# balisujohn/tortoise.cpp

Measured on AMD Instinct MI355X. Metric: audio-seconds/sec end-to-end (AR+diffusion+vocoder), 16 cands x 80 steps, higher is better.
Workload: dtype f16 MFMA inputs / f32 accumulate (diffusion, vocoder convs); f32 weights, f16 KV (AR)

## Files before the change

### tortoise.cpp_amd/csrc/api.cpp

```cpp
#include "common.h"
#include <sched.h>
#include <cctype>
#include <cmath>
#include <algorithm>
#include <chrono>
#include <fstream>
#include <new>

namespace tts {
int ar_begin(tts_ctx *, const int32_t *, int, const float *, int, int);
int ar_begin_groups(tts_ctx *, const int32_t *, const int *, int, const float *, int n_voices, const int *voice_of, const int *, int);
int ar_latents_group(tts_ctx *, int, const int32_t *, int, float *);
int ar_prefill(tts_ctx *, float *);
int ar_step(tts_ctx *, const int32_t *, int, float *, int mode);
const int32_t *ar_host_lists(tts_ctx *);
const float *ar_fetch_logits_row(tts_ctx *, int);
int ar_batch(const tts_ctx *);
int ar_latents(tts_ctx *, const int32_t *, int, int, float *);
int ar_layers(const tts_ctx *);
float *ar_host_logits(tts_ctx *);
int diff_layers(const tts_ctx *);
int diff_forward(tts_ctx *, const float *, int, const float *, int, int, float *);
int diff_sample(tts_ctx *, const float *, const int32_t *, int, int, const float *, int, float *);
int diff_sample_voices(tts_ctx *, const float *, const int32_t *, int, const float *, int, const int32_t *, int, const float *, int, float *);
// ... 113 lines not shown
  for (hipEvent_t e : c->ev_pool) (void)hipEventDestroy(e);
  if (c->ev0) (void)hipEventDestroy(c->ev0);
  if (c->ev1) (void)hipEventDestroy(c->ev1);
  if (c->stream) (void)hipStreamDestroy(c->stream);
  if (c->load_stream) (void)hipStreamDestroy(c->load_stream);
  delete c;
}

int tts_version(void) { return TTS_API_VERSION; }

const char *tts_last_error(const tts_ctx *c) { return c ? c->err.c_str() : "no context (no HIP device?)"; }

int tts_set_option(tts_ctx *c, const char *key, double value) {
  if (!c || !key) return TTS_ERR_ARG;
  std::string k(key);
  if (k == "gn_eps") c->gn_eps = (float)value;
  else if (k == "ggml_lut") c->ggml_lut = value != 0;
  else if (k.rfind("prof_only:", 0) == 0) {
    if (value != 0) c->prof_filter.push_back(k.substr(10));
    else c->prof_filter.clear();
  }
  else if (k == "device_topk") c->device_topk = value != 0;
  else if (k == "sampler_threads") {
    if (c->sampler_pool) { sampler_pool_free(c->sampler_pool); c->sampler_pool = nullptr; }
    c->sampler_threads = value < 0 ? -1 : (int)value;
  }
  else if (k == "share_uncond") c->share_uncond = value != 0;
  else if (k == "prof_stride") c->prof_stride = value < 1 ? 1 : (int)value;
  else if (k == "diff_graph") c->diff_graph = value != 0;
  else if (k == "dec_f32_mfma") c->dec_f32_mfma = value != 0;
  else if (k == "attn_f32") c->attn_f32 = value != 0;
  else if (k == "attn_proj_f16") c->attn_proj_f16 = value != 0;
  else if (k == "proj_dual_b") c->proj_dual_b = value != 0;
  else if (k == "gemm_wreg") c->gemm_wreg = value == 1 ? tts_ctx::GEMM_WREG_ALL : value == 2 ? 1 : value == 3 ? 2 : 0;
  else if (k == "lc_attn_f32") c->lc_attn_f32 = value != 0;
  else if (k == "latency_mode") c->latency_mode = value != 0;
  else if (k == "fp16_check") c->fp16_check = value != 0;
  else if (k == "rng_fast_normal") c->rng_fast_normal = value != 0;
  else if (k == "noise_pipeline") c->noise_pipeline = value != 0;
  else if (k == "load_device_pack") c->load_device_pack = value != 0;
  else if (k == "load_threads") c->load_threads = value < 0 ? 0 : value > 64 ? 64 : (int)value;
  else if (k == "attn_q64") c->attn_q64 = value < 0 ? 0 : value > 2 ? 2 : (int)value;
  else if (k == "hoist_integrator") c->hoist_integrator = value < 0 ? 0 : (int)value;
  else if (k == "attn_f32_drop") c->attn_f32_drop = (int)value & 7;
  else if (k == "ar_weights") {
    if (value != 0 && value != 1 && value != 2) return fail(c, TTS_ERR_ARG, "ar_weights: 0 (f32), 1 (fp16) or 2 (fp8 e4m3)");
    c->ar_weights = (int)value;
  }
  else if (k == "diff_sampler") {
    if (value != 0 && value != 1) return fail(c, TTS_ERR_ARG, "diff_sampler: 0 (ancestral DDPM) or 1 (DDIM)");
    c->diff_sampler = (int)value;
  }
  else if (k == "ddim_eta") {
    if (!(value >= 0 && value <= 1)) return fail(c, TTS_ERR_ARG, "ddim_eta: a value in [0, 1]");
    c->ddim_eta = value;
  }
  else if (k == "cond_free_k") {
    if (!std::isfinite(value) || value < 0 || !std::isfinite((float)value)) return fail(c, TTS_ERR_ARG, "cond_free_k: a finite value >= 0");
    c->cond_free_k = (float)value;
  }
  else if (k == "prof_eager_every") c->prof_eager_every = value < 1 ? 1 : (int)value;
  else if (k == "stream_cus") {
    if (c->device < 0) return fail(c, TTS_ERR_HIP, "host-only context: no stream");
    if (c->ar || c->diff || c->voc || c->clvp || c->venc || c->dcond) return fail(c, TTS_ERR_STATE, "stream_cus must be set before the models are loaded");
    (void)hipSetDevice(c->device);
    hipDeviceProp_t prop;
    if (hipGetDeviceProperties(&prop, c->device) != hipSuccess) return fail(c, TTS_ERR_HIP, "hipGetDeviceProperties failed");
// ... 435 lines not shown
```

### tortoise.cpp_amd/csrc/common.h

```cpp
#pragma once
#include "../../include/tortoise_mi355x.h"
#include <hip/hip_runtime.h>
#include <cstdarg>
#include <cstdint>
#include <cstdio>
#include <cstring>
#include <functional>
#include <map>
#include <memory>
#include <random>
#include <algorithm>
#include <atomic>
#include <condition_variable>
#include <mutex>
#include <new>
#include <string>
#include <thread>
#include <vector>

namespace tts {

struct HostTensor {
  std::vector<float> data;
  int64_t ne[4] = {1, 1, 1, 1};
// ... 67 lines not shown
  int device = 0;
  hipStream_t stream = nullptr;
  hipStream_t load_stream = nullptr;
  int stream_cus = 0;
  std::string err;
  float gn_eps = 1e-6f;
  int ggml_lut = 0;
  std::mt19937 generator;
  std::uniform_real_distribution<float> distribution{0.0, 1.0};
  std::normal_distribution<double> normal_distribution{0.0, 1.0};
  uint32_t seed_value = 0;
  tts::ArState *ar = nullptr;
  tts::DiffState *diff = nullptr;
  tts::VocState *voc = nullptr;
  tts::ClvpState *clvp = nullptr;
  tts::VoiceEncState *venc = nullptr;
  tts::DiffCondEncState *dcond = nullptr;
  tts::Tokenizer *tok = nullptr;
  tts::SamplerPool *sampler_pool = nullptr;
  int device_topk = 1;
  int time_mlp_retries = 0;
  int topk_fallbacks = 0;
  int sampler_threads = -1;
  bool share_uncond = true;
  int rng_shard_offset = 0, rng_shard_total = 0;
  std::vector<int32_t> stop_schedule;
  std::vector<int32_t> ar_stopped;
  bool prof_on = false;
  std::vector<std::string> prof_filter;
  int prof_stride = 1;
  int ar_weights = 0;
  int dec_f32_mfma = 0;
  int attn_f32 = 0;
  static constexpr int GEMM_WREG_ALL = 3;
  int gemm_wreg = GEMM_WREG_ALL;
  int proj_dual_b = 1;
  int attn_f32_drop = 0;
  int lc_attn_f32 = 1;
  int attn_proj_f16 = 0;
  int fp16_check = 0;
  int64_t fp16_bad_weights[2] = {0, 0};
  void *fp16_counts = nullptr;
  int rng_fast_normal = 1;
  int noise_pipeline = 1;
  int load_device_pack = 1;
  int load_threads = 0;
  int attn_q64 = 0;
  int hoist_integrator = 1;
  int latency_mode = 0;
  int diff_sampler = 0;
  double ddim_eta = 0;
  float cond_free_k = 2.0f;
  bool capturing = false;
  int diff_graph = 1;
  int prof_eager_every = 8;
  std::map<std::string, tts::ProfEntry> prof;
  std::vector<hipEvent_t> ev_pool;
  hipEvent_t ev0 = nullptr, ev1 = nullptr;
};

namespace tts {

int fail(tts_ctx *ctx, int code, const char *fmt, ...);

void rng_normal_fill(tts_ctx *ctx, float *dst, int64_t n);

struct PinnedPool {
// ... 178 lines not shown
```

### tortoise.cpp_amd/csrc/diffusion.hip

```cpp
#include "common.h"
#include "gemm_f16.h"
#include <algorithm>
#include <chrono>
#include <cmath>

namespace tts {

static constexpr int C = 1024, NHEAD = 16, XTC = 128 ;
static constexpr int LAT_MAX_ROWS = 2048;
static constexpr int HOIST_MAX_ROWS = 16384;

__device__ __forceinline__ float silu_dev(float x, int lut) {
  if (lut == 1) {
    float xr = __half2float(__float2half_rn(x));
    return __half2float(__float2half_rn(xr / (1.0f + expf(-xr))));
  }
  if (lut == 2) return x / (1.0f + expf(-x));
  return x * __builtin_amdgcn_rcpf(1.0f + __builtin_amdgcn_exp2f(x * -1.44269504088896f));
}

__global__ __launch_bounds__(256) void gn_stats_kernel(const float *__restrict__ x, const int *__restrict__ seq_start,
                                                       const int *__restrict__ seq_len, float eps, float2 *__restrict__ stats) {
  __shared__ float sh[8];
  const int grp = blockIdx.x, s = blockIdx.y, T = seq_len[s];
// ... 667 lines not shown
    const float xs = sc.sqrt_recip * xv;
    float x0 = xs - sc.sqrt_recipm1 * eps_g;
    x0 = fminf(fmaxf(x0, -1.0f), 1.0f);
    const float eps_h = (xs - x0) / sc.sqrt_recipm1;
    outv = d.c_x0 * x0 + d.c_eps * eps_h;
    if (!sc.is_last && d.sigma != 0.0f) {
      const float nz = noise ? noise[xi] : philox_normal(seed, stream0 + (uint32_t)s, e.philox_step, (uint32_t)(ch * T + t));
      outv = outv + d.sigma * nz;
    }
  }
  x[xi] = outv;
}

__global__ void philox_fill_kernel(float *__restrict__ x, int64_t n, uint64_t seed, uint32_t stream, uint32_t step) {
  int64_t i = (int64_t)blockIdx.x * blockDim.x + threadIdx.x;
  if (i < n) x[i] = philox_normal(seed, stream, step, (uint32_t)i);
}

__global__ void rows_to_ct_kernel(const float *__restrict__ net, int row0, int T, int nch, int ld, float *__restrict__ out) {
  int i = blockIdx.x * blockDim.x + threadIdx.x;
  if (i < nch * T) {
    int ch = i / T, t = i - ch * T;
    out[i] = net[(size_t)(row0 + t) * ld + ch];
  }
}

struct AttnDev {
  float *norm_g, *norm_b, *qkv_b, *proj_b, *bias_tab;
  __half *qkv_w, *proj_w;
  __half *qkv_wf;
  __half *proj_w_split;
  float proj_alpha;
};
struct ResDev { float *in_g, *in_b, *in_bias, *emb_w, *emb_b, *out_g, *out_b, *out_bias; __half *in_w, *out_w, *in_wf; };

struct Layout {
  int ns = 0, rows = 0;
  std::vector<int> start, len;
  DevBuf d_row_seq, d_row_t, d_start, d_len, d_chunk_seq;
  int build(tts_ctx *ctx, const std::vector<int> &lens) {
    has_seq_step = false; ss_step_stride = 0;
    ns = (int)lens.size();
    len = lens;
    start.resize(ns);
    int r = 8;
    for (int s = 0; s < ns; s++) { start[s] = r; r = (r + lens[s] + 1 + 7) & ~7; }
    rows = (r + 127) & ~127;
    std::vector<int> rs(rows, -1), rt(rows, 0);
    for (int s = 0; s < ns; s++)
      for (int t = 0; t < lens[s]; t++) { rs[start[s] + t] = s; rt[start[s] + t] = t; }
    TTS_HIP(ctx, d_row_seq.reserve(rows * 4)); TTS_HIP(ctx, d_row_t.reserve(rows * 4));
    TTS_HIP(ctx, d_start.reserve(ns * 4)); TTS_HIP(ctx, d_len.reserve(ns * 4));
    TTS_HIP(ctx, hipMemcpy(d_row_seq.p, rs.data(), rows * 4, hipMemcpyHostToDevice));
    TTS_HIP(ctx, hipMemcpy(d_row_t.p, rt.data(), rows * 4, hipMemcpyHostToDevice));
    TTS_HIP(ctx, hipMemcpy(d_start.p, start.data(), ns * 4, hipMemcpyHostToDevice));
    TTS_HIP(ctx, hipMemcpy(d_len.p, len.data(), ns * 4, hipMemcpyHostToDevice));
    std::vector<int> cs(rows / 8, -1);
    for (int s = 0; s < ns; s++)
      for (int t = 0; t < lens[s]; t++) cs[(start[s] + t) >> 3] = s;
    TTS_HIP(ctx, d_chunk_seq.reserve(rows / 8 * 4));
    TTS_HIP(ctx, hipMemcpy(d_chunk_seq.p, cs.data(), rows / 8 * 4, hipMemcpyHostToDevice));
    return TTS_OK;
  }
  int max_len() const { return len.empty() ? 0 : *std::max_element(len.begin(), len.end()); }
  DevBuf d_seq_step;
  int ss_step_stride = 0;
  bool has_seq_step = false;
// ... 100 lines not shown
    if (it->second.nelem() != nelem) {
      fail(ctx, TTS_ERR_FORMAT, "tensor '%s' has wrong size in model file: got %lld, expected %lld", name.c_str(),
           (long long)it->second.nelem(), (long long)nelem);
      return nullptr;
    }
    { std::lock_guard<std::mutex> lk(mu); used[name] = true; }
    return &it->second;
  }
  template <class T> int put(const std::vector<T> &h, T **dst) {
    void *p = nullptr;
    TTS_HIP(ctx, hipMalloc(&p, h.size() * sizeof(T)));
    { std::lock_guard<std::mutex> lk(mu); st->owned.push_back(p); }
    TTS_HIP(ctx, pin.upload(p, h.data(), h.size() * sizeof(T), ctx->load_stream));
    *dst = (T *)p;
    return TTS_OK;
  }
  int f32(const std::string &name, int64_t n, float **dst) {
    const HostTensor *t = get(name, n);
    if (!t) return TTS_ERR_FORMAT;
    return put(t->data, dst);
  }
  int conv16(const std::string &name, int cout, int cin, int k, int cout_pad, int cin_pad, __half **dst, __half **dst_frag = nullptr) {
    const HostTensor *t = get(name, (int64_t)cout * cin * k);
    if (!t) return TTS_ERR_FORMAT;
    std::vector<__half> h((size_t)cout_pad * k * cin_pad, __float2half(0.f));
    const float *w = t->data.data();
    for (int co = 0; co < cout; co++)
      for (int ci = 0; ci < cin; ci++)
        for (int tap = 0; tap < k; tap++)
          h[(size_t)co * k * cin_pad + (size_t)tap * cin_pad + ci] = __float2half_rn(w[((size_t)co * cin + ci) * k + tap]);
    if (dst_frag) {
      std::vector<__half> f(h.size());
      for (int n = 0; n < cout_pad; n++)
        for (int c = 0; c < cin_pad; c++) f[gemm_wfrag_index(n, c, cin_pad)] = h[(size_t)n * cin_pad + c];
      if (int r = put(f, dst_frag)) return r;
    }
    return put(h, dst);
  }
  int attn(const std::string &p, AttnDev &a) {
    int r;
    if ((r = f32(p + ".norm.weight", C, &a.norm_g))) return r;
    if ((r = f32(p + ".norm.bias", C, &a.norm_b))) return r;
    if ((r = conv16(p + ".qkv.weight", 3 * C, C, 1, 3 * C, C, &a.qkv_w, &a.qkv_wf))) return r;
    if ((r = f32(p + ".qkv.bias", 3 * C, &a.qkv_b))) return r;
    if ((r = conv16(p + ".proj_out.weight", C, C, 1, C, C, &a.proj_w))) return r;
    {
      const HostTensor *t = get(p + ".proj_out.weight", (int64_t)C * C);
      std::vector<__half> sp((size_t)C * 2 * C);
      float amax = 0.f;
      for (float v : t->data) amax = std::max(amax, std::fabs(v));
      if (!std::isfinite(amax)) { fail(ctx, TTS_ERR_FORMAT, "tensor '%s.proj_out.weight' holds a non-finite value", p.c_str()); return TTS_ERR_FORMAT; }
      int e = 14;
      while (e > -14 && std::ldexp(amax, e) >= 30000.0f) e--;
      const float scale = std::ldexp(1.0f, e);
      a.proj_alpha = 1.0f / scale;
      for (int n = 0; n < C; n++)
        for (int k = 0; k < C; k++) {
          const float w = t->data[(size_t)n * C + k] * scale;
          const __half hi = __float2half_rn(w);
          sp[(size_t)n * 2 * C + k] = hi;
          sp[(size_t)n * 2 * C + C + k] = __float2half_rn(w - __half2float(hi));
        }
      long long bad[2] = {0, 0};
      for (const __half &h : sp) {
        const float v = std::fabs(__half2float(h));
        if (!(v <= 65504.0f)) bad[0]++;
        else if (v > 60000.0f) bad[1]++;
      }
      if (bad[0] | bad[1]) { std::lock_guard<std::mutex> lk(mu); ctx->fp16_bad_weights[0] += bad[0]; ctx->fp16_bad_weights[1] += bad[1]; }
      if ((r = put(sp, &a.proj_w_split))) return r;
    }
    if ((r = f32(p + ".proj_out.bias", C, &a.proj_b))) return r;
    const HostTensor *t = get(p + ".relative_pos_embeddings.relative_attention_bias.weight", 32 * 16);
    if (!t) return TTS_ERR_FORMAT;
    std::vector<float> tab(16 * 128);
    for (int h = 0; h < 16; h++)
      for (int sgn = 0; sgn < 2; sgn++)
        for (int d = 0; d < 64; d++) {
          int bucket = sgn ? rel_bucket(0, d) : rel_bucket(d, 0);
          if (d == 0) bucket = rel_bucket(0, 0);
          tab[h * 128 + sgn * 64 + d] = t->data[(size_t)bucket * 16 + h] * 8.0f;
        }
    return put(tab, &a.bias_tab);
  }
  int res(const std::string &p, ResDev &w) {
    int r;
    if ((r = f32(p + ".in_layers.0.weight", C, &w.in_g))) return r;
    if ((r = f32(p + ".in_layers.0.bias", C, &w.in_b))) return r;
    if ((r = conv16(p + ".in_layers.2.weight", C, C, 1, C, C, &w.in_w, &w.in_wf))) return r;
    if ((r = f32(p + ".in_layers.2.bias", C, &w.in_bias))) return r;
    if ((r = f32(p + ".emb_layers.1.weight", 2 * C * C, &w.emb_w))) return r;
    if ((r = f32(p + ".emb_layers.1.bias", 2 * C, &w.emb_b))) return r;
    if ((r = f32(p + ".out_layers.0.weight", C, &w.out_g))) return r;
    if ((r = f32(p + ".out_layers.0.bias", C, &w.out_b))) return r;
    if ((r = conv16(p + ".out_layers.3.weight", C, C, 3, C, C, &w.out_w))) return r;
    if ((r = f32(p + ".out_layers.3.bias", C, &w.out_bias))) return r;
    return TTS_OK;
  }
};
}

int diff_load(tts_ctx *ctx, const char *path) {
  ctx->fp16_bad_weights[0] = ctx->fp16_bad_weights[1] = 0;
  WeightFile wf;
  std::string err;
  int rc = read_weight_file(path, wf, err);
  if (rc != TTS_OK) return fail(ctx, rc, "diffusion_model_load: %s", err.c_str());
  std::unique_ptr<DiffState> st(new DiffState());
  Loader ld{ctx, st.get(), wf, {}};
  while (wf.has("latent_conditioner." + std::to_string(st->n_lc + 1) + ".norm.weight")) st->n_lc++;
  while (wf.has("conditioning_timestep_integrator." + std::to_string(st->n_integ) + ".resblk.in_layers.0.weight")) st->n_integ++;
  while (wf.has("layers." + std::to_string(st->n_main) + ".resblk.in_layers.0.weight")) st->n_main++;
  while (wf.has("layers." + std::to_string(st->n_main + st->n_tail) + ".in_layers.0.weight")) st->n_tail++;
  st->lc_attn.resize(st->n_lc);
  st->integ_res.resize(st->n_integ); st->integ_attn.resize(st->n_integ);
  st->main_res.resize(st->n_main); st->main_attn.resize(st->n_main);
  st->tail_res.resize(st->n_tail);
  std::vector<std::function<int()>> jobs;
  DiffState *S = st.get();
#define J(x) jobs.emplace_back([&ld, S]() -> int { (void)S; return (x); })
  J(ld.f32("diffusion_conditioning_latent", 2 * C, &S->cond_latent));
  J(ld.f32("unconditioned_embedding", C, &S->uncond_emb));
  J(ld.conv16("latent_conditioner.0.weight", C, C, 3, C, C, &S->lc_w));
  J(ld.f32("latent_conditioner.0.bias", C, &S->lc_bias));
  for (int i = 0; i < st->n_lc; i++) jobs.emplace_back([&ld, S, i]() { return ld.attn("latent_conditioner." + std::to_string(i + 1), S->lc_attn[i]); });
  J(ld.f32("code_norm.weight", C, &S->code_g));
  J(ld.f32("code_norm.bias", C, &S->code_b));
  J(ld.f32("time_embed.0.weight", C * C, &S->te0_w)); J(ld.f32("time_embed.0.bias", C, &S->te0_b));
// ... 393 lines not shown
    return gemm(ctx, "diff_gemm", p, lay, 0, C);
  }
  if (!ctx->attn_proj_f16) {
    GemmArgs p = gemm_base(lay, wk.ATT16(), C, 2, C, w.proj_w_split, C, w.proj_b);
    p.custom_w = 1; p.ldw_ = 2 * C; p.w_off_[0] = 0; p.w_off_[1] = C;
    p.mode = st_out ? GEMM_OUT_F32_SCALED_STATS : GEMM_OUT_F32_SCALED; p.alpha = w.proj_alpha; p.outF = X; p.ldo = C; p.resid = X;
    p.st_out = st_out; p.st_stripe_ll = (int)st->gn_stripe_ll; p.chunk_seq = lay.d_chunk_seq.as<int>();
    p.dual_b = ctx->proj_dual_b;
    CHECK(gemm(ctx, "diff_gemm", p, lay, 0, C));
    DBG_SUM("attn proj", X, (size_t)lay.rows * C * 4);
    return TTS_OK;
  }
  GemmArgs p = gemm_base(lay, wk.ATT16(), C, 1, C, w.proj_w, C, w.proj_b);
  p.mode = st_out ? GEMM_OUT_F32_STATS : GEMM_OUT_F32; p.outF = X; p.ldo = C; p.resid = X;
  p.st_out = st_out; p.st_stripe_ll = (int)st->gn_stripe_ll; p.chunk_seq = lay.d_chunk_seq.as<int>();
  CHECK(gemm(ctx, "diff_gemm", p, lay));
  DBG_SUM("attn proj", X, (size_t)lay.rows * C * 4);
  return TTS_OK;
}

static int res_block(tts_ctx *ctx, DiffState *st, const Layout &lay, Work &wk, float *X, const ResDev &w, const float *ss,
                     const float *Xin = nullptr, const float *Hpre = nullptr, const long long *st_hpre = nullptr) {
  const float *xin = Xin ? Xin : X;
  const bool lat = st->lat && (Hpre ? st_hpre != nullptr : wk.st_x != nullptr);
  const long long *st_h = st_hpre;
  if (!Hpre) {
    long long *slot = lat ? st->new_stats_slot() : nullptr;
    CHECK(res_in_layers(ctx, st, lay, wk, xin, w, wk.H(), lat ? wk.st_x : nullptr, slot));
    Hpre = wk.H();
    st_h = slot;
  }
  DBG_SUM("res.out ss", ss, (size_t)2 * C * 4);
  DBG_SUM("res.out hpre", Hpre, (size_t)lay.rows * C * 4);
  CHECK(gn(ctx, st, lay, Hpre, lat ? st_h : nullptr, w.out_g, w.out_b, ss, 1, wk.A16(), w.out_w, (size_t)3 * C * C * 2));
  DBG_SUM("res.out gn", wk.A16(), (size_t)lay.rows * C * 2);
  GemmArgs c3 = gemm_base(lay, wk.A16(), C, 3, C, w.out_w, C, w.out_bias);
  long long *st_out = lat ? st->new_stats_slot() : nullptr;
  c3.mode = st_out ? GEMM_OUT_F32_STATS : GEMM_OUT_F32; c3.outF = X; c3.ldo = C; c3.resid = xin;
  c3.st_out = st_out; c3.st_stripe_ll = (int)st->gn_stripe_ll; c3.chunk_seq = lay.d_chunk_seq.as<int>();
  wk.st_x = st_out;
  CHECK(gemm(ctx, "diff_gemm", c3, lay));
  DBG_SUM("res.out conv", X, (size_t)lay.rows * C * 4);
  return TTS_OK;
}

template <int CTRL> __device__ __forceinline__ float lnk_dpp(float x) {
  return __int_as_float(__builtin_amdgcn_update_dpp(0, __float_as_int(x), CTRL, 0xf, 0xf, false));
}
__device__ __forceinline__ float wave_sum_dpp(float x) {
  auto a = __builtin_amdgcn_permlane32_swap(__float_as_uint(x), __float_as_uint(x), false, false);
  x = __uint_as_float(a[0]) + __uint_as_float(a[1]);
  auto b = __builtin_amdgcn_permlane16_swap(__float_as_uint(x), __float_as_uint(x), false, false);
  x = __uint_as_float(b[0]) + __uint_as_float(b[1]);
  x += lnk_dpp<0x128>(x);
  x += lnk_dpp<0x124>(x);
  x += lnk_dpp<0x122>(x);
  x += lnk_dpp<0x121>(x);
  return x;
}

static constexpr int LNK_COLS = 32;
static __global__ __launch_bounds__(1024) void linear_nk_kernel(const float *__restrict__ x, int ldx, int rows, const float *__restrict__ W,
                                                         int N, const float *__restrict__ b, float *__restrict__ out, int ldo,
                                                         int act ) {
  const int lane = threadIdx.x & 63;
  for (int half = 0; half < 2; half++) {
    const int n = blockIdx.x * LNK_COLS + half * 16 + (threadIdx.x >> 6);
    if (n >= N) return;
    const float *wr = W + (size_t)n * C + lane * 4;
// ... 504 lines not shown
```

### tortoise.cpp_amd/csrc/gemm_f16.h

```cpp
#pragma once
#include <hip/hip_fp16.h>
#include <hip/hip_runtime.h>
#include <algorithm>
#include <cmath>
#include <cstdlib>
#include <type_traits>

namespace tts {

typedef _Float16 half8 __attribute__((ext_vector_type(8)));
typedef float floatx4 __attribute__((ext_vector_type(4)));

enum { GEMM_OUT_F32 = 0, GEMM_OUT_F16 = 1, GEMM_OUT_QKV = 2, GEMM_OUT_QKV_SPLIT = 3, GEMM_OUT_F32_SCALED = 4, GEMM_OUT_F32_STATS = 5, GEMM_OUT_F32_SCALED_STATS = 6 };
constexpr bool gemm_mode_qkv(int mode) { return mode == GEMM_OUT_QKV || mode == GEMM_OUT_QKV_SPLIT; }
constexpr bool gemm_mode_f32(int mode) { return mode == GEMM_OUT_F32 || mode == GEMM_OUT_F32_SCALED || mode == GEMM_OUT_F32_STATS || mode == GEMM_OUT_F32_SCALED_STATS; }
constexpr bool gemm_mode_scaled(int mode) { return mode == GEMM_OUT_F32_SCALED || mode == GEMM_OUT_F32_SCALED_STATS; }
constexpr bool gemm_mode_stats(int mode) { return mode == GEMM_OUT_F32_STATS || mode == GEMM_OUT_F32_SCALED_STATS; }

struct GemmArgs {
  const __half *A[3];
  int row_off[3];
  int nseg, kseg;
  int lda;
  const __half *W;
// ... 698 lines not shown
#pragma unroll
        for (int j = 0; j < 4; j++) acc[i][j] = __builtin_amdgcn_mfma_f32_16x16x32_f16(bf[j], af[i], acc[i][j], 0, 0, 0);
    }
    asm volatile("s_waitcnt lgkmcnt(0)" ::: "memory");
    __builtin_amdgcn_s_barrier();
    if (TAP == 2) stageA(kc + 1);
  };
  stageA(0);
  stageB(0);
  for (int kc = 0; kc < nchunks; kc++) {
    const int p = 3 * kc;
    phase(kc, p, std::integral_constant<int, 0>{});
    phase(kc, p + 1, std::integral_constant<int, 1>{});
    phase(kc, p + 2, std::integral_constant<int, 2>{});
  }
  asm volatile("s_waitcnt vmcnt(0)" ::: "memory");
  if ((MODE == GEMM_OUT_F32 || MODE == GEMM_OUT_F32_STATS) && g.resid) gemm_epilogue_vh<MODE, MI, EPI_RESID_LOAD>(g, acc, m0, n0, wm, wn, fr, fq);
  else gemm_epilogue_vh<MODE, MI, EPI_NO_RESID>(g, acc, m0, n0, wm, wn, fr, fq);
}

template <int MODE>
static __global__ __launch_bounds__(256, 3) void gemm_f16_conv3_vh_kernel(GemmArgs g) {
  const int tid = threadIdx.x, lane = tid & 63, wave = __builtin_amdgcn_readfirstlane(tid >> 6);
  int m0, n0, nblk;
  if (!gemm_vh_tile(g, m0, n0, nblk)) return;
  gemm_for_my_mi(nblk, wave, [&](auto mi) { gemm_conv3_vh_body<MODE, decltype(mi)::value>(g, m0, n0, nblk, lane, wave); });
}

static inline bool gemm_is_conv3(const GemmArgs &g) {
  return g.nseg == 3 && !g.custom_w && g.A[0] == g.A[1] && g.A[1] == g.A[2] && g.row_off[0] == -1 && g.row_off[1] == 0 && g.row_off[2] == 1 &&
         !gemm_mode_qkv(g.mode) && !gemm_mode_scaled(g.mode);
}

static inline int gemm_auto_th(int M, int N) {
  const int maxb = ((M >> 4) + 7) / 8 + 1, NT = N >> 7;
  int th = 2;
  while (th < 8 && 8 * ((maxb + th - 1) / th) * NT > 1024) th *= 2;
  return th;
}

enum { GEMM_KERNEL_VH = 0, GEMM_KERNEL_DUALB = 1, GEMM_KERNEL_CONV3 = 2, GEMM_KERNEL_WREG = 3 };
struct GemmPlan {
  hipError_t err;
  int kernel;
  int th, ku, cn;
  int grid, lds;
};
static inline GemmPlan gemm_plan(const GemmArgs &g) {
  GemmPlan p = {};
  const int NT = g.N >> 7, ktot = g.nseg * g.kseg, nb = g.M >> 4;
  p.err = hipSuccess;
  if (gemm_mode_scaled(g.mode)) {
    int e;
    if (!(g.alpha != 0.f) || std::fabs(std::frexp(g.alpha, &e)) != 0.5f) p.err = hipErrorInvalidValue;
  }
  if (gemm_mode_stats(g.mode) && (!g.st_out || !g.chunk_seq || g.st_stripe_ll <= 0)) p.err = hipErrorInvalidValue;
  if (g.dual_b && !(gemm_mode_scaled(g.mode) && g.nseg == 2 && g.custom_w && g.A[0] == g.A[1] && g.row_off[0] == g.row_off[1])) p.err = hipErrorInvalidValue;
  int ku = (g.ku == 2 || g.ku == 4) && (g.kseg % (64 * g.ku)) == 0 ? g.ku : 1;
  p.cn = NT;
  if (NT > 8)
    for (p.cn = NT; p.cn > 1; p.cn--)
      if (NT % p.cn == 0 && (size_t)p.cn * 128 * ktot * 2 <= (size_t)2560 * 1024) break;
  const int maxb = (nb + 7) / 8 + 1;
  p.th = g.th > 0 ? g.th : gemm_auto_th(g.M, g.N);
  if (g.th <= 0 && g.ku == 0 && NT <= 8 && 8 * ((maxb + 3) / 4) * NT <= 256 && (g.kseg % 256) == 0) {
    p.th = 4;
    if (!gemm_is_conv3(g)) ku = g.dual_b ? 2 : 4;
  }
  int mt_max = 0;
  for (int x = 0; x < 8; x++) {
    const int b0 = (int)((long long)nb * x >> 3), b1 = (int)((long long)nb * (x + 1) >> 3);
    mt_max = std::max(mt_max, (b1 - b0 + p.th - 1) / p.th);
  }
  p.grid = 8 * mt_max * NT;
  if (gemm_takes_wreg(g, p.th, ku)) { p.kernel = GEMM_KERNEL_WREG; p.ku = 1; p.lds = GEMM_WREG_LDS; }
  else if (gemm_is_conv3(g)) { p.kernel = GEMM_KERNEL_CONV3; p.ku = 1; p.lds = CONV3_VH_LDS; }
  else if (g.dual_b) { p.kernel = GEMM_KERNEL_DUALB; p.ku = ku == 2 ? 2 : 1; p.lds = p.ku * GEMM_DUALB_LDS; }
  else { p.kernel = GEMM_KERNEL_VH; p.ku = ku; p.lds = ku * GEMM_VH_LDS; }
  return p;
}

static_assert(GEMM_DUALB_LDS <= 48 * 1024 && GEMM_VH_LDS <= 48 * 1024 && GEMM_WREG_LDS <= 48 * 1024 && CONV3_VH_LDS > 48 * 1024, "which launches raise their dynamic LDS limit");
template <void (*KERN)(GemmArgs)> static inline void gemm_launch(const GemmPlan &p, const GemmArgs &g, hipStream_t s) {
  if (p.lds > 48 * 1024) {
    static bool raised = false;
    if (!raised) { (void)hipFuncSetAttribute((const void *)KERN, hipFuncAttributeMaxDynamicSharedMemorySize, p.lds); raised = true; }
  }
  KERN<<<p.grid, 256, p.lds, s>>>(g);
}
template <int KU> static inline void gemm_launch_vh(const GemmPlan &p, const GemmArgs &g, hipStream_t s) {
  constexpr int WGS = KU == 1 ? 4 : KU == 2 ? 2 : 1;
  switch (g.mode) {
    case GEMM_OUT_F32: return gemm_launch<gemm_f16_vh_kernel<GEMM_OUT_F32, WGS, KU>>(p, g, s);
    case GEMM_OUT_F16: return gemm_launch<gemm_f16_vh_kernel<GEMM_OUT_F16, WGS, KU>>(p, g, s);
    case GEMM_OUT_QKV: return gemm_launch<gemm_f16_vh_kernel<GEMM_OUT_QKV, WGS, KU>>(p, g, s);
    case GEMM_OUT_QKV_SPLIT: return gemm_launch<gemm_f16_vh_kernel<GEMM_OUT_QKV_SPLIT, WGS, KU>>(p, g, s);
    case GEMM_OUT_F32_SCALED: return gemm_launch<gemm_f16_vh_kernel<GEMM_OUT_F32_SCALED, WGS, KU>>(p, g, s);
    case GEMM_OUT_F32_STATS: return gemm_launch<gemm_f16_vh_kernel<GEMM_OUT_F32_STATS, WGS, KU>>(p, g, s);
    default: return gemm_launch<gemm_f16_vh_kernel<GEMM_OUT_F32_SCALED_STATS, WGS, KU>>(p, g, s);
  }
}
template <int KU> static inline void gemm_launch_dualb(const GemmPlan &p, const GemmArgs &g, hipStream_t s) {
  if (g.mode == GEMM_OUT_F32_SCALED) gemm_launch<gemm_f16_vh_dualb_kernel<GEMM_OUT_F32_SCALED, KU>>(p, g, s);
  else gemm_launch<gemm_f16_vh_dualb_kernel<GEMM_OUT_F32_SCALED_STATS, KU>>(p, g, s);
}
static inline void gemm_launch_conv3(const GemmPlan &p, const GemmArgs &g, hipStream_t s) {
  if (g.mode == GEMM_OUT_F32) gemm_launch<gemm_f16_conv3_vh_kernel<GEMM_OUT_F32>>(p, g, s);
  else if (g.mode == GEMM_OUT_F32_STATS) gemm_launch<gemm_f16_conv3_vh_kernel<GEMM_OUT_F32_STATS>>(p, g, s);
  else gemm_launch<gemm_f16_conv3_vh_kernel<GEMM_OUT_F16>>(p, g, s);
}
static inline void gemm_launch_wreg(const GemmPlan &p, const GemmArgs &g, hipStream_t s) {
  if (g.mode == GEMM_OUT_F32) gemm_launch<gemm_f16_wreg_kernel<GEMM_OUT_F32>>(p, g, s);
  else if (g.mode == GEMM_OUT_QKV) gemm_launch<gemm_f16_wreg_kernel<GEMM_OUT_QKV>>(p, g, s);
  else gemm_launch<gemm_f16_wreg_kernel<GEMM_OUT_QKV_SPLIT>>(p, g, s);
}

static inline hipError_t launch_gemm_f16(const GemmArgs &g, hipStream_t s) {
  const GemmPlan p = gemm_plan(g);
  if (p.err != hipSuccess) return p.err;
  GemmArgs gg = g;
  gg.th = p.th;
  gg.cn = p.cn;
  if (p.kernel == GEMM_KERNEL_WREG) gemm_launch_wreg(p, gg, s);
  else if (p.kernel == GEMM_KERNEL_CONV3) gemm_launch_conv3(p, gg, s);
  else if (p.kernel == GEMM_KERNEL_DUALB) p.ku == 2 ? gemm_launch_dualb<2>(p, gg, s) : gemm_launch_dualb<1>(p, gg, s);
  else p.ku == 4 ? gemm_launch_vh<4>(p, gg, s) : p.ku == 2 ? gemm_launch_vh<2>(p, gg, s) : gemm_launch_vh<1>(p, gg, s);
  return hipGetLastError();
}

}
```

### tortoise.cpp_amd/testlib/gemm_harness.hip

```cpp
#include "../csrc/gemm_f16.h"

#include <cstdint>
#include <cstdio>
#include <cstring>
#include <vector>

using namespace tts;

extern "C" {

enum { TTS_GEMM_TEST_MARGIN = 4096, TTS_GEMM_TEST_SENTINEL = 0xCB };

struct tts_gemm_case {
  int M, N, nseg, kseg;
  int row_off[3], a_sel[3];
  int mode, th, ku, wreg, dual_b, custom_w, ldw, w_off[3];
  float alpha;
  int has_bias, has_resid, resid_aliases_out, has_row_seq, has_chunk_seq, has_st;
  int lda, ldo, ldh, ldvt, nseq, st_stripe_ll, launches;
  const uint16_t *A0, *A1, *W;
  const float *bias, *resid;
  const int *row_seq, *chunk_seq;
  float *outF;
  uint16_t *outH, *outH2, *outVt, *outVt2;
  long long *st;
};

int tts_gemm_test_margin(void) { return TTS_GEMM_TEST_MARGIN; }
int tts_gemm_test_auto_th(int M, int N) { return gemm_auto_th(M, N); }

}

namespace {

char g_last[160] = "none";

GemmArgs host_args(const tts_gemm_case &c) {
  static const __half dummy[2] = {};
  GemmArgs g;
  memset(&g, 0, sizeof g);
  for (int s = 0; s < 3; s++) {
    g.A[s] = dummy + (c.a_sel[s] ? 1 : 0);
    g.row_off[s] = c.row_off[s];
    g.w_off_[s] = c.w_off[s];
  }
  g.nseg = c.nseg; g.kseg = c.kseg; g.lda = c.lda; g.custom_w = c.custom_w; g.ldw_ = c.ldw;
  g.wreg = c.wreg; g.M = c.M; g.N = c.N; g.ldo = c.ldo; g.ldh = c.ldh; g.ldvt = c.ldvt; g.alpha = c.alpha;
  g.st_stripe_ll = c.st_stripe_ll; g.dual_b = c.dual_b; g.mode = c.mode; g.th = c.th; g.ku = c.ku;
  return g;
}

void describe(const GemmArgs &g, char *buf, int cap) {
  static const char *const names[] = {"vh", "dualb", "conv3", "wreg"};
  const GemmPlan p = gemm_plan(g);
  snprintf(buf, cap, "%s mode=%d th=%d ku=%d cn=%d", names[p.kernel], g.mode, p.th, p.ku, p.cn);
}

struct Dev {
  char *p = nullptr;
  size_t bytes = 0;
  ~Dev() { if (p) (void)hipFree(p); }
  hipError_t alloc(size_t payload, int fill) {
    bytes = payload;
    hipError_t e = hipMalloc((void **)&p, payload + 2 * TTS_GEMM_TEST_MARGIN);
    if (e != hipSuccess) { p = nullptr; return e; }
    return hipMemset(p, fill, payload + 2 * TTS_GEMM_TEST_MARGIN);
  }
  char *data() const { return p + TTS_GEMM_TEST_MARGIN; }
  hipError_t put(const void *h) { return hipMemcpy(data(), h, bytes, hipMemcpyHostToDevice); }
  hipError_t get_all(void *h) const { return hipMemcpy(h, p, bytes + 2 * TTS_GEMM_TEST_MARGIN, hipMemcpyDeviceToHost); }
};

bool valid(const tts_gemm_case &c, bool run) {
  if (c.M < 16 || c.M > 131072 || (c.M & 15) || c.N < 128 || c.N > 4096 || (c.N & 127)) return false;
  if (c.nseg < 1 || c.nseg > 3 || c.kseg < 64 || c.kseg > 4096 || (c.kseg & 63)) return false;
  if (c.mode < GEMM_OUT_F32 || c.mode > GEMM_OUT_F32_SCALED_STATS || c.th < 0 || c.th > 8) return false;
  if (!(c.ku == 0 || c.ku == 1 || c.ku == 2 || c.ku == 4) || c.launches < 1 || c.launches > 2) return false;
  if (c.lda < c.kseg || c.lda < 64 || (c.lda & 7) || !c.A0 || !c.W) return false;
  for (int s = 0; s < c.nseg; s++) {
    if (c.row_off[s] < -1 || c.row_off[s] > 1) return false;
    if (c.a_sel[s] != 0 && c.a_sel[s] != 1) return false;
    if (c.a_sel[s] == 1 && !c.A1) return false;
  }
  const int ldw = c.custom_w ? c.ldw : c.nseg * c.kseg;
  if (ldw < 64 || (ldw & 7)) return false;
  for (int s = 0; s < c.nseg; s++) {
    const int off = c.custom_w ? c.w_off[s] : s * c.kseg;
    if (off < 0 || (off & 7) || off + c.kseg > ldw) return false;
  }
  if (c.has_bias && !c.bias) return false;
  if (c.has_row_seq && !c.row_seq) return false;
  if (c.has_resid && (!gemm_mode_f32(c.mode) || (!c.resid_aliases_out && !c.resid))) return false;
  if (c.resid_aliases_out && !(c.has_resid && c.resid)) return false;
  if (gemm_mode_f32(c.mode)) {
    if ((run && !c.outF) || c.ldo < c.N || (c.ldo & 3)) return false;
  } else if (c.mode == GEMM_OUT_F16) {
    if ((run && !c.outH) || c.ldh < c.N || (c.ldh & 3)) return false;
  } else {
    if (c.N % 384) return false;
    if ((run && (!c.outH || !c.outVt)) || c.ldh < c.N / 192 * 128 || (c.ldh & 3) || c.ldvt < c.M || (c.ldvt & 3)) return false;
    if (run && c.mode == GEMM_OUT_QKV_SPLIT && (!c.outH2 || !c.outVt2)) return false;
  }
  if (gemm_mode_stats(c.mode) && (c.has_st || c.has_chunk_seq)) {
    if (c.N > 1024 || c.nseq < 1) return false;
    if (c.has_st && ((run && !c.st) || (c.st_stripe_ll > 0 && c.st_stripe_ll < c.nseq * 32 * 4))) return false;
    if (c.has_chunk_seq) {
      if (!c.chunk_seq) return false;
      for (int i = 0; i < c.M / 8; i++)
        if (c.chunk_seq[i] < -1 || c.chunk_seq[i] >= c.nseq) return false;
    }
  }
  return true;
}

}

extern "C" {

int tts_gemm_test_plan(const tts_gemm_case *c, char *buf, int cap) {
  if (!c || !buf || cap <= 0 || !valid(*c, false)) return (int)hipErrorInvalidValue;
  GemmArgs g = host_args(*c);
  static const __half wf_placeholder[1] = {};
  if (c->wreg && c->nseg == 1 && !c->custom_w) g.Wf = wf_placeholder;
  describe(g, buf, cap);
  return 0;
}

int tts_gemm_test_last_kernel(char *buf, int cap) {
  if (!buf || cap <= 0) return (int)hipErrorInvalidValue;
  snprintf(buf, cap, "%s", g_last);
  return 0;
}

#define HT(x) do { hipError_t e_ = (x); if (e_ != hipSuccess) return (int)e_; } while (0)

int tts_gemm_test_run(const tts_gemm_case *cp) {
  if (!cp || !valid(*cp, true)) return (int)hipErrorInvalidValue;
  const tts_gemm_case &c = *cp;
  const int ldw = c.custom_w ? c.ldw : c.nseg * c.kseg;
  const size_t a_bytes = (size_t)(c.M + 2) * c.lda * 2, w_bytes = (size_t)c.N * ldw * 2;
  const size_t f_bytes = (size_t)c.M * c.ldo * 4, h_bytes = (size_t)c.M * c.ldh * 2, vt_bytes = (size_t)(c.N / 192 * 64) * c.ldvt * 2;
  const size_t st_bytes = (size_t)FX_STRIPES * (c.st_stripe_ll > 0 ? c.st_stripe_ll : 0) * 8;
  Dev a0, a1, w, wf, bias, resid, rseq, cseq, outF, outH, outH2, outVt, outVt2, st;
  GemmArgs g = host_args(c);
  HT(a0.alloc(a_bytes, 0)); HT(a0.put(c.A0));
  if (c.A1) { HT(a1.alloc(a_bytes, 0)); HT(a1.put(c.A1)); }
  HT(w.alloc(w_bytes, 0)); HT(w.put(c.W));
  for (int s = 0; s < 3; s++) g.A[s] = (const __half *)((c.a_sel[s] && s < c.nseg ? a1 : a0).data()) + c.lda;
  g.W = (const __half *)w.data();
  if (c.wreg && c.nseg == 1 && !c.custom_w) {
    std::vector<uint16_t> img((size_t)c.N * c.kseg);
    for (int n = 0; n < c.N; n++)
      for (int k = 0; k < c.kseg; k++) img[gemm_wfrag_index(n, k, c.kseg)] = c.W[(size_t)n * c.kseg + k];
    HT(wf.alloc(w_bytes, 0)); HT(wf.put(img.data()));
    g.Wf = (const __half *)wf.data();
  }
  if (c.has_bias) { HT(bias.alloc((size_t)c.N * 4, 0)); HT(bias.put(c.bias)); g.bias = (const float *)bias.data(); }
  if (c.has_row_seq) { HT(rseq.alloc((size_t)c.M * 4, 0xFF)); HT(rseq.put(c.row_seq)); g.row_seq = (const int *)rseq.data(); }
  if (gemm_mode_f32(c.mode)) {
    HT(outF.alloc(f_bytes, TTS_GEMM_TEST_SENTINEL));
    g.outF = (float *)outF.data();
    if (c.has_resid && c.resid_aliases_out) { HT(outF.put(c.resid)); g.resid = g.outF; }
    else if (c.has_resid) { HT(resid.alloc(f_bytes, 0)); HT(resid.put(c.resid)); g.resid = (const float *)resid.data(); }
  } else {
    HT(outH.alloc(h_bytes, TTS_GEMM_TEST_SENTINEL));
    g.outH = (__half *)outH.data();
    if (gemm_mode_qkv(c.mode)) { HT(outVt.alloc(vt_bytes, TTS_GEMM_TEST_SENTINEL)); g.outVt = (__half *)outVt.data(); }
    if (c.mode == GEMM_OUT_QKV_SPLIT) {
      HT(outH2.alloc(h_bytes, TTS_GEMM_TEST_SENTINEL)); HT(outVt2.alloc(vt_bytes, TTS_GEMM_TEST_SENTINEL));
      g.outH2 = (__half *)outH2.data(); g.outVt2 = (__half *)outVt2.data();
    }
  }
  if (gemm_mode_stats(c.mode)) {
    if (c.has_st && st_bytes) {
      HT(st.alloc(st_bytes, TTS_GEMM_TEST_SENTINEL)); HT(hipMemset(st.data(), 0, st_bytes));
      g.st_out = (long long *)st.data();
    }
    if (c.has_chunk_seq) { HT(cseq.alloc((size_t)c.M / 8 * 4, 0xFF)); HT(cseq.put(c.chunk_seq)); g.chunk_seq = (const int *)cseq.data(); }
  }
  describe(g, g_last, sizeof g_last);
  hipStream_t s;
  HT(hipStreamCreateWithFlags(&s, hipStreamNonBlocking));
  hipError_t e = hipDeviceSynchronize();
  for (int l = 0; l < c.launches && e == hipSuccess; l++) e = launch_gemm_f16(g, s);
  const hipError_t es = hipStreamSynchronize(s);
  (void)hipStreamDestroy(s);
  if (outF.p) HT(outF.get_all(c.outF));
  if (outH.p) HT(outH.get_all(c.outH));
  if (outH2.p) HT(outH2.get_all(c.outH2));
  if (outVt.p) HT(outVt.get_all(c.outVt));
  if (outVt2.p) HT(outVt2.get_all(c.outVt2));
  if (st.p) HT(st.get_all(c.st));
  return (int)(e != hipSuccess ? e : es);
}

}
```

Before: 135.1.

## Add register-resident weight kernel for diffusion resblock output conv3 GEMM

```diff
diff --git a/tortoise.cpp_amd/csrc/api.cpp b/tortoise.cpp_amd/csrc/api.cpp
--- a/tortoise.cpp_amd/csrc/api.cpp
+++ b/tortoise.cpp_amd/csrc/api.cpp
@@ -169,7 +169,7 @@
   else if (k == "attn_f32") c->attn_f32 = value != 0;
   else if (k == "attn_proj_f16") c->attn_proj_f16 = value != 0;
   else if (k == "proj_dual_b") c->proj_dual_b = value != 0;
-  else if (k == "gemm_wreg") c->gemm_wreg = value == 1 ? tts_ctx::GEMM_WREG_ALL : value == 2 ? 1 : value == 3 ? 2 : 0;
+  else if (k == "gemm_wreg") c->gemm_wreg = value == 1 ? tts_ctx::GEMM_WREG_ALL : value == 2 ? 1 : value == 3 ? 2 : value == 4 ? 4 : 0;
   else if (k == "lc_attn_f32") c->lc_attn_f32 = value != 0;
   else if (k == "latency_mode") c->latency_mode = value != 0;
   else if (k == "fp16_check") c->fp16_check = value != 0;
diff --git a/tortoise.cpp_amd/csrc/common.h b/tortoise.cpp_amd/csrc/common.h
--- a/tortoise.cpp_amd/csrc/common.h
+++ b/tortoise.cpp_amd/csrc/common.h
@@ -123,7 +123,7 @@
   int ar_weights = 0;
   int dec_f32_mfma = 0;
   int attn_f32 = 0;
-  static constexpr int GEMM_WREG_ALL = 3;
+  static constexpr int GEMM_WREG_ALL = 7;
   int gemm_wreg = GEMM_WREG_ALL;
   int proj_dual_b = 1;
   int attn_f32_drop = 0;
diff --git a/tortoise.cpp_amd/csrc/diffusion.hip b/tortoise.cpp_amd/csrc/diffusion.hip
--- a/tortoise.cpp_amd/csrc/diffusion.hip
+++ b/tortoise.cpp_amd/csrc/diffusion.hip
@@ -723,7 +723,7 @@
   __half *proj_w_split;
   float proj_alpha;
 };
-struct ResDev { float *in_g, *in_b, *in_bias, *emb_w, *emb_b, *out_g, *out_b, *out_bias; __half *in_w, *out_w, *in_wf; };
+struct ResDev { float *in_g, *in_b, *in_bias, *emb_w, *emb_b, *out_g, *out_b, *out_bias; __half *in_w, *out_w, *in_wf, *out_wf; };
 
 struct Layout {
   int ns = 0, rows = 0;
@@ -890,7 +890,8 @@
     if (dst_frag) {
       std::vector<__half> f(h.size());
       for (int n = 0; n < cout_pad; n++)
-        for (int c = 0; c < cin_pad; c++) f[gemm_wfrag_index(n, c, cin_pad)] = h[(size_t)n * cin_pad + c];
+        for (int tap = 0; tap < k; tap++)
+          for (int c = 0; c < cin_pad; c++) f[gemm_wfrag3_index(n, tap, c, cout_pad, cin_pad)] = h[((size_t)n * k + tap) * cin_pad + c];
       if (int r = put(f, dst_frag)) return r;
     }
     return put(h, dst);
@@ -951,7 +952,7 @@
     if ((r = f32(p + ".emb_layers.1.bias", 2 * C, &w.emb_b))) return r;
     if ((r = f32(p + ".out_layers.0.weight", C, &w.out_g))) return r;
     if ((r = f32(p + ".out_layers.0.bias", C, &w.out_b))) return r;
-    if ((r = conv16(p + ".out_layers.3.weight", C, C, 3, C, C, &w.out_w))) return r;
+    if ((r = conv16(p + ".out_layers.3.weight", C, C, 3, C, C, &w.out_w, &w.out_wf))) return r;
     if ((r = f32(p + ".out_layers.3.bias", C, &w.out_bias))) return r;
     return TTS_OK;
   }
@@ -1411,9 +1412,10 @@
   }
   DBG_SUM("res.out ss", ss, (size_t)2 * C * 4);
   DBG_SUM("res.out hpre", Hpre, (size_t)lay.rows * C * 4);
-  CHECK(gn(ctx, st, lay, Hpre, lat ? st_h : nullptr, w.out_g, w.out_b, ss, 1, wk.A16(), w.out_w, (size_t)3 * C * C * 2));
+  CHECK(gn(ctx, st, lay, Hpre, lat ? st_h : nullptr, w.out_g, w.out_b, ss, 1, wk.A16(), lat ? w.out_w : gemm_wreg_image(ctx, 4, lay, C, w.out_w, w.out_wf), (size_t)3 * C * C * 2));
   DBG_SUM("res.out gn", wk.A16(), (size_t)lay.rows * C * 2);
   GemmArgs c3 = gemm_base(lay, wk.A16(), C, 3, C, w.out_w, C, w.out_bias);
+  c3.Wf = w.out_wf; c3.wreg = gemm_wreg_class(ctx, 4);
   long long *st_out = lat ? st->new_stats_slot() : nullptr;
   c3.mode = st_out ? GEMM_OUT_F32_STATS : GEMM_OUT_F32; c3.outF = X; c3.ldo = C; c3.resid = xin;
   c3.st_out = st_out; c3.st_stripe_ll = (int)st->gn_stripe_ll; c3.chunk_seq = lay.d_chunk_seq.as<int>();
diff --git a/tortoise.cpp_amd/csrc/gemm_f16.h b/tortoise.cpp_amd/csrc/gemm_f16.h
--- a/tortoise.cpp_amd/csrc/gemm_f16.h
+++ b/tortoise.cpp_amd/csrc/gemm_f16.h
@@ -754,6 +754,169 @@
          !gemm_mode_qkv(g.mode) && !gemm_mode_scaled(g.mode);
 }
 
+static inline size_t gemm_wfrag3_index(int n, int tap, int k, int N, int K) {
+  return (size_t)tap * N * K + gemm_wfrag_index(n, k, K);
+}
+static constexpr int CONV3_WREG_SLOT = (128 + 8) * 128, CONV3_WREG_LDS = 2 * CONV3_WREG_SLOT;
+
+template <int MI, bool RESID>
+__device__ __forceinline__ void gemm_epilogue_conv3_wreg(const GemmArgs &g, floatx4 (&acc)[MI][2], int m0, int n0, int nblk, int wave, int fr, int fq) {
+  const int col0 = n0 + wave * 32 + fq * 4;
+  const bool hb = g.bias != nullptr, hs = g.row_seq != nullptr;
+  const float *bp = hb ? g.bias : (const float *)g.W;
+  const int *sp = hs ? g.row_seq : (const int *)g.A[0];
+  float4 b4[2], rr[2][2];
+  int sq[MI];
+  auto load_pair = [&](int p) {
+#pragma unroll
+    for (int q = 0; q < 2; q++) {
+      const float *rp = g.resid + (size_t)(m0 + min(2 * p + q, nblk - 1) * 16 + fr) * g.ldo + col0;
+#pragma unroll
+      for (int j = 0; j < 2; j++) rr[q][j] = *(const float4 *)(rp + j * 16);
+    }
+  };
+  if (RESID) load_pair(0);
+#pragma unroll
+  for (int j = 0; j < 2; j++) b4[j] = *(const float4 *)(bp + col0 + j * 16);
+#pragma unroll
+  for (int i = 0; i < MI; i++) sq[i] = sp[m0 + min(i, nblk - 1) * 16 + fr];
+#pragma unroll
+  for (int j = 0; j < 2; j++) b4[j] = hb ? b4[j] : make_float4(0.f, 0.f, 0.f, 0.f);
+#pragma unroll
+  for (int i = 0; i < MI; i++) sq[i] = hs ? sq[i] : 0;
+#pragma unroll
+  for (int p = 0; p < MI / 2; p++) {
+    float4 v[2][2];
+#pragma unroll
+    for (int q = 0; q < 2; q++) {
+      const int i = 2 * p + q;
+#pragma unroll
+      for (int j = 0; j < 2; j++) {
+        float4 t = make_float4(acc[i][j][0] + b4[j].x, acc[i][j][1] + b4[j].y, acc[i][j][2] + b4[j].z, acc[i][j][3] + b4[j].w);
+        if (RESID) { t.x += rr[q][j].x; t.y += rr[q][j].y; t.z += rr[q][j].z; t.w += rr[q][j].w; }
+        if (sq[i] < 0) t = make_float4(0.f, 0.f, 0.f, 0.f);
+        v[q][j] = t;
+      }
+    }
+    if (RESID && p + 1 < MI / 2) load_pair(p + 1);
+#pragma unroll
+    for (int q = 0; q < 2; q++) {
+      const int i = 2 * p + q;
+      if (i < nblk) {
+        float *op = g.outF + (size_t)(m0 + i * 16 + fr) * g.ldo + col0;
+#pragma unroll
+        for (int j = 0; j < 2; j++) *(float4 *)(op + j * 16) = v[q][j];
+      }
+    }
+  }
+}
+
+template <int MI, bool RESID>
+__device__ __forceinline__ void gemm_conv3_wreg_body(const GemmArgs &g, int m0, int n0, int nblk, int lane, int wave) {
+  extern __shared__ __attribute__((aligned(16))) char smem_dyn[];
+  char *smem = smem_dyn;
+  constexpr int NP = 2 * MI + 1;
+  constexpr int NPA = (NP + 3) / 4;
+  const int nchunks = g.kseg >> 6, KS = g.kseg >> 5;
+  const int fr = lane & 15, fq = lane >> 4;
+  unsigned aoff[NPA];
+#pragma unroll
+  for (int i = 0; i < NPA; i++) aoff[i] = (unsigned)(gemm_dma_off(min(wave + 4 * i, NP - 1), lane, 0, nblk * 16 + 1, g.lda) * 2);
+  const char *aseg = (const char *)(g.A[0] + (ptrdiff_t)(m0 - 1) * g.lda);
+  const size_t tap_stride = (size_t)g.N * g.kseg;
+  const __half *wp = g.Wf + (size_t)((n0 >> 4) + wave * 2) * KS * 512;
+  const unsigned wlane = lane * 16;
+  floatx4 acc[MI][2];
+#pragma unroll
+  for (int i = 0; i < MI; i++)
+#pragma unroll
+    for (int j = 0; j < 2; j++) acc[i][j] = (floatx4){0.f, 0.f, 0.f, 0.f};
+  int fbase[3][2];
+#pragma unroll
+  for (int tap = 0; tap < 3; tap++)
+#pragma unroll
+    for (int ks = 0; ks < 2; ks++) {
+      fbase[tap][ks] = lds_off(fr + tap, ks * 4 + fq);
+      asm volatile("" : "+v"(fbase[tap][ks]));
+    }
+  half8 w[2][2][2];
+  auto issue_w = [&](int kc, int tap, auto set_c) {
+    constexpr int U = decltype(set_c)::value;
+    const __half *q0 = wp + (size_t)tap * tap_stride + (size_t)min(kc, nchunks - 1) * 1024, *q1 = q0 + (size_t)KS * 512;
+    wreg_load<0>(w[U][0][0], q0, wlane);
+    wreg_load<0>(w[U][0][1], q1, wlane);
+    wreg_load<1024>(w[U][1][0], q0, wlane);
+    wreg_load<1024>(w[U][1][1], q1, wlane);
+  };
+  auto issue_slab = [&](int kc, int slot) {
+    const char *ab = aseg + (min(kc, nchunks - 1) << 7);
+    asm volatile("" : "+s"(ab));
+#pragma unroll
+    for (int i = 0; i < NPA; i++) {
+      unsigned o = aoff[i];
+      asm volatile("" : "+v"(o));
+      __builtin_amdgcn_global_load_lds((gptr_t)(ab + o), (lptr_t)(smem + slot * CONV3_WREG_SLOT + min(wave + 4 * i, NP - 1) * 1024), 16, 0, 0);
+    }
+  };
+  auto phase = [&](int kc, auto par_c, auto tap_c) {
+    constexpr int PAR = decltype(par_c)::value, TAP = decltype(tap_c)::value, U = PAR ^ (TAP & 1);
+    wreg_wait<TAP == 1 ? NPA : 0>(w[U][0][0], w[U][0][1], w[U][1][0], w[U][1][1]);
+    if (TAP == 0) {
+      asm volatile("s_waitcnt lgkmcnt(0)" ::: "memory");
+      __builtin_amdgcn_s_barrier();
+    }
+    if (TAP < 2) issue_w(kc, TAP + 1, std::integral_constant<int, U ^ 1>{});
+    else issue_w(kc + 1, 0, std::integral_constant<int, U ^ 1>{});
+    if (TAP == 0) issue_slab(kc + 1, PAR ^ 1);
+    const char *sa = smem + PAR * CONV3_WREG_SLOT;
+    constexpr int AHEAD = 2;
+    half8 af[AHEAD + 1];
+    auto frag = [&](int x) { return *(const half8 *)(sa + fbase[TAP][x / MI] + (x % MI) * 2048); };
+#pragma unroll
+    for (int x = 0; x < AHEAD; x++) af[x] = frag(x);
+#pragma unroll
+    for (int x = 0; x < 2 * MI; x++) {
+      if (x + AHEAD < 2 * MI) af[(x + AHEAD) % (AHEAD + 1)] = frag(x + AHEAD);
+      const int ks = x / MI, i = x % MI;
+      const half8 a = af[x % (AHEAD + 1)];
+#pragma unroll
+      for (int j = 0; j < 2; j++) acc[i][j] = __builtin_amdgcn_mfma_f32_16x16x32_f16(w[U][ks][j], a, acc[i][j], 0, 0, 0);
+    }
+    __builtin_amdgcn_sched_group_barrier(0x100, AHEAD, 0);
+#pragma unroll
+    for (int x = 0; x < 2 * MI; x++) {
+      if (x + AHEAD < 2 * MI) __builtin_amdgcn_sched_group_barrier(0x100, 1, 0);
+      __builtin_amdgcn_sched_group_barrier(0x008, 2, 0);
+    }
+  };
+  auto chunk = [&](int kc, auto par_c) {
+    phase(kc, par_c, std::integral_constant<int, 0>{});
+    phase(kc, par_c, std::integral_constant<int, 1>{});
+    phase(kc, par_c, std::integral_constant<int, 2>{});
+  };
+  issue_slab(0, 0);
+  issue_w(0, 0, std::integral_constant<int, 0>{});
+  for (int kc = 0; kc < nchunks; kc += 2) {
+    chunk(kc, std::integral_constant<int, 0>{});
+    if (kc + 1 < nchunks) chunk(kc + 1, std::integral_constant<int, 1>{});
+  }
+  wreg_wait<0>(w[0][0][0], w[0][0][1], w[0][1][0], w[0][1][1]);
+  wreg_wait<0>(w[1][0][0], w[1][0][1], w[1][1][0], w[1][1][1]);
+  gemm_epilogue_conv3_wreg<MI, RESID>(g, acc, m0, n0, nblk, wave, fr, fq);
+}
+
+template <bool RESID>
+static __global__ __launch_bounds__(256, 4) void gemm_f16_conv3_wreg_kernel(GemmArgs g) {
+  const int tid = threadIdx.x, lane = tid & 63, wave = __builtin_amdgcn_readfirstlane(tid >> 6);
+  int m0, n0, nblk;
+  if (!gemm_vh_tile(g, m0, n0, nblk)) return;
+  if (nblk > 4) gemm_conv3_wreg_body<8, RESID>(g, m0, n0, nblk, lane, wave);
+  else gemm_conv3_wreg_body<4, RESID>(g, m0, n0, nblk, lane, wave);
+}
+static inline bool gemm_takes_conv3_wreg(const GemmArgs &g, int th) {
+  return g.wreg > 0 && g.Wf && gemm_is_conv3(g) && th == 8 && g.mode == GEMM_OUT_F32;
+}
+
 static inline int gemm_auto_th(int M, int N) {
   const int maxb = ((M >> 4) + 7) / 8 + 1, NT = N >> 7;
   int th = 2;
@@ -761,7 +924,7 @@
   return th;
 }
 
-enum { GEMM_KERNEL_VH = 0, GEMM_KERNEL_DUALB = 1, GEMM_KERNEL_CONV3 = 2, GEMM_KERNEL_WREG = 3 };
+enum { GEMM_KERNEL_VH = 0, GEMM_KERNEL_DUALB = 1, GEMM_KERNEL_CONV3 = 2, GEMM_KERNEL_WREG = 3, GEMM_KERNEL_CONV3_WREG = 4 };
 struct GemmPlan {
   hipError_t err;
   int kernel;
@@ -796,13 +959,14 @@
   }
   p.grid = 8 * mt_max * NT;
   if (gemm_takes_wreg(g, p.th, ku)) { p.kernel = GEMM_KERNEL_WREG; p.ku = 1; p.lds = GEMM_WREG_LDS; }
+  else if (gemm_takes_conv3_wreg(g, p.th)) { p.kernel = GEMM_KERNEL_CONV3_WREG; p.ku = 1; p.lds = CONV3_WREG_LDS; }
   else if (gemm_is_conv3(g)) { p.kernel = GEMM_KERNEL_CONV3; p.ku = 1; p.lds = CONV3_VH_LDS; }
   else if (g.dual_b) { p.kernel = GEMM_KERNEL_DUALB; p.ku = ku == 2 ? 2 : 1; p.lds = p.ku * GEMM_DUALB_LDS; }
   else { p.kernel = GEMM_KERNEL_VH; p.ku = ku; p.lds = ku * GEMM_VH_LDS; }
   return p;
 }
 
-static_assert(GEMM_DUALB_LDS <= 48 * 1024 && GEMM_VH_LDS <= 48 * 1024 && GEMM_WREG_LDS <= 48 * 1024 && CONV3_VH_LDS > 48 * 1024, "which launches raise their dynamic LDS limit");
+static_assert(GEMM_DUALB_LDS <= 48 * 1024 && GEMM_VH_LDS <= 48 * 1024 && GEMM_WREG_LDS <= 48 * 1024 && CONV3_WREG_LDS <= 48 * 1024 && CONV3_VH_LDS > 48 * 1024, "which launches raise their dynamic LDS limit");
 template <void (*KERN)(GemmArgs)> static inline void gemm_launch(const GemmPlan &p, const GemmArgs &g, hipStream_t s) {
   if (p.lds > 48 * 1024) {
     static bool raised = false;
@@ -831,6 +995,10 @@
   else if (g.mode == GEMM_OUT_F32_STATS) gemm_launch<gemm_f16_conv3_vh_kernel<GEMM_OUT_F32_STATS>>(p, g, s);
   else gemm_launch<gemm_f16_conv3_vh_kernel<GEMM_OUT_F16>>(p, g, s);
 }
+static inline void gemm_launch_conv3_wreg(const GemmPlan &p, const GemmArgs &g, hipStream_t s) {
+  if (g.resid) gemm_launch<gemm_f16_conv3_wreg_kernel<true>>(p, g, s);
+  else gemm_launch<gemm_f16_conv3_wreg_kernel<false>>(p, g, s);
+}
 static inline void gemm_launch_wreg(const GemmPlan &p, const GemmArgs &g, hipStream_t s) {
   if (g.mode == GEMM_OUT_F32) gemm_launch<gemm_f16_wreg_kernel<GEMM_OUT_F32>>(p, g, s);
   else if (g.mode == GEMM_OUT_QKV) gemm_launch<gemm_f16_wreg_kernel<GEMM_OUT_QKV>>(p, g, s);
@@ -844,6 +1012,7 @@
   gg.th = p.th;
   gg.cn = p.cn;
   if (p.kernel == GEMM_KERNEL_WREG) gemm_launch_wreg(p, gg, s);
+  else if (p.kernel == GEMM_KERNEL_CONV3_WREG) gemm_launch_conv3_wreg(p, gg, s);
   else if (p.kernel == GEMM_KERNEL_CONV3) gemm_launch_conv3(p, gg, s);
   else if (p.kernel == GEMM_KERNEL_DUALB) p.ku == 2 ? gemm_launch_dualb<2>(p, gg, s) : gemm_launch_dualb<1>(p, gg, s);
   else p.ku == 4 ? gemm_launch_vh<4>(p, gg, s) : p.ku == 2 ? gemm_launch_vh<2>(p, gg, s) : gemm_launch_vh<1>(p, gg, s);
diff --git a/tortoise.cpp_amd/testlib/gemm_harness.hip b/tortoise.cpp_amd/testlib/gemm_harness.hip
--- a/tortoise.cpp_amd/testlib/gemm_harness.hip
+++ b/tortoise.cpp_amd/testlib/gemm_harness.hip
@@ -28,6 +28,7 @@
 
 int tts_gemm_test_margin(void) { return TTS_GEMM_TEST_MARGIN; }
 int tts_gemm_test_auto_th(int M, int N) { return gemm_auto_th(M, N); }
+long long tts_gemm_test_wfrag3_index(int n, int tap, int k, int N, int K) { return (long long)gemm_wfrag3_index(n, tap, k, N, K); }
 
 }
 
@@ -51,7 +52,7 @@
 }
 
 void describe(const GemmArgs &g, char *buf, int cap) {
-  static const char *const names[] = {"vh", "dualb", "conv3", "wreg"};
+  static const char *const names[] = {"vh", "dualb", "conv3", "wreg", "conv3w"};
   const GemmPlan p = gemm_plan(g);
   snprintf(buf, cap, "%s mode=%d th=%d ku=%d cn=%d", names[p.kernel], g.mode, p.th, p.ku, p.cn);
 }
@@ -70,6 +71,10 @@
   hipError_t put(const void *h) { return hipMemcpy(data(), h, bytes, hipMemcpyHostToDevice); }
   hipError_t get_all(void *h) const { return hipMemcpy(h, p, bytes + 2 * TTS_GEMM_TEST_MARGIN, hipMemcpyDeviceToHost); }
 };
+
+bool conv3_shape(const tts_gemm_case &c) {
+  return c.nseg == 3 && !c.custom_w && !c.a_sel[0] && !c.a_sel[1] && !c.a_sel[2] && c.row_off[0] == -1 && c.row_off[1] == 0 && c.row_off[2] == 1;
+}
 
 bool valid(const tts_gemm_case &c, bool run) {
   if (c.M < 16 || c.M > 131072 || (c.M & 15) || c.N < 128 || c.N > 4096 || (c.N & 127)) return false;
@@ -117,14 +122,16 @@
 
 extern "C" {
 
-int tts_gemm_test_plan(const tts_gemm_case *c, char *buf, int cap) {
+static int plan_case(const tts_gemm_case *c, char *buf, int cap, bool images) {
   if (!c || !buf || cap <= 0 || !valid(*c, false)) return (int)hipErrorInvalidValue;
   GemmArgs g = host_args(*c);
   static const __half wf_placeholder[1] = {};
-  if (c->wreg && c->nseg == 1 && !c->custom_w) g.Wf = wf_placeholder;
+  if (c->wreg && ((c->nseg == 1 && !c->custom_w) || (images && conv3_shape(*c)))) g.Wf = wf_placeholder;
   describe(g, buf, cap);
   return 0;
 }
+int tts_gemm_test_plan(const tts_gemm_case *c, char *buf, int cap) { return plan_case(c, buf, cap, false); }
+int tts_gemm_test_plan_images(const tts_gemm_case *c, char *buf, int cap) { return plan_case(c, buf, cap, true); }
 
 int tts_gemm_test_last_kernel(char *buf, int cap) {
   if (!buf || cap <= 0) return (int)hipErrorInvalidValue;
@@ -134,7 +141,7 @@
 
 #define HT(x) do { hipError_t e_ = (x); if (e_ != hipSuccess) return (int)e_; } while (0)
 
-int tts_gemm_test_run(const tts_gemm_case *cp) {
+static int run_case(const tts_gemm_case *cp, bool images) {
   if (!cp || !valid(*cp, true)) return (int)hipErrorInvalidValue;
   const tts_gemm_case &c = *cp;
   const int ldw = c.custom_w ? c.ldw : c.nseg * c.kseg;
@@ -154,6 +161,13 @@
       for (int k = 0; k < c.kseg; k++) img[gemm_wfrag_index(n, k, c.kseg)] = c.W[(size_t)n * c.kseg + k];
     HT(wf.alloc(w_bytes, 0)); HT(wf.put(img.data()));
     g.Wf = (const __half *)wf.data();
+  } else if (images && c.wreg && conv3_shape(c)) {
+    std::vector<uint16_t> img((size_t)c.N * 3 * c.kseg);
+    for (int n = 0; n < c.N; n++)
+      for (int tap = 0; tap < 3; tap++)
+        for (int k = 0; k < c.kseg; k++) img[gemm_wfrag3_index(n, tap, k, c.N, c.kseg)] = c.W[((size_t)n * 3 + tap) * c.kseg + k];
+    HT(wf.alloc(w_bytes, 0)); HT(wf.put(img.data()));
+    g.Wf = (const __half *)wf.data();
   }
   if (c.has_bias) { HT(bias.alloc((size_t)c.N * 4, 0)); HT(bias.put(c.bias)); g.bias = (const float *)bias.data(); }
   if (c.has_row_seq) { HT(rseq.alloc((size_t)c.M * 4, 0xFF)); HT(rseq.put(c.row_seq)); g.row_seq = (const int *)rseq.data(); }
@@ -194,4 +208,7 @@
   return (int)(e != hipSuccess ? e : es);
 }
 
-}
+int tts_gemm_test_run(const tts_gemm_case *cp) { return run_case(cp, false); }
+int tts_gemm_test_run_images(const tts_gemm_case *cp) { return run_case(cp, true); }
+
+}
```

Result: faster. 136.9 (median of 6 runs) (+1.3%).
